# YAIconvalley/distributed-pipeline

Measured on AMD Instinct MI355X. Metric: train steps/sec (whole node), DiffuSeq-base seq128 DDP at 1/2/4/8 MI355X, higher is better.
Workload: dtype bf16

## Files before the change

distributed_pipeline_amd/csrc/bindings.cpp:

```cpp
#include <cstdlib>
#include <cstring>
#include <torch/extension.h>
#include <ATen/hip/impl/HIPStreamMasqueradingAsCUDA.h>
#include <c10/core/DeviceGuard.h>

#include <vector>

#include "launchers.h"

namespace dpa {
void register_comm(pybind11::module& m);
void register_runtime(pybind11::module& m);
}

#define CHECK_DEV(x) TORCH_CHECK((x).is_cuda(), #x " must be a HIP tensor")
#define CHECK_CONTIG(x) TORCH_CHECK((x).is_contiguous(), #x " must be contiguous")
#define CHECK_F32(x) TORCH_CHECK((x).scalar_type() == at::kFloat, #x " must be float32")
#define CHECK_BF16(x) TORCH_CHECK((x).scalar_type() == at::kBFloat16, #x " must be bfloat16")
#define CHECK_ALIGNED(x) \
  TORCH_CHECK(reinterpret_cast<uintptr_t>((x).data_ptr()) % 16 == 0, #x " must be 16-byte aligned")

static inline hipStream_t cur_stream() { return c10::hip::getCurrentHIPStreamMasqueradingAsCUDA().stream(); }

static void sqnorm(const at::Tensor& g, at::Tensor& partial, at::Tensor& out, double scale,
// ... 1207 lines not shown
        py::arg("part_buf") = py::none(), py::arg("part_acc") = false, py::arg("beta") = py::none(),
        py::arg("hcopy") = py::none(), py::arg("pair_hash") = false);
  m.def("colsum_acc", &colsum_acc, "dst += colsum(part) (fp32 partials [rows, cols])");
  m.def("ln_bwd_partials", &ln_bwd_partials, "floats of add_ln_bwd's deferred partial buffer (0: none)");
  m.def("ln_colreduce", &ln_colreduce, "dg/db(/dyb) += column sums of add_ln_bwd partials",
        py::arg("part"), py::arg("R"), py::arg("D"), py::arg("dg"), py::arg("db"), py::arg("dyb") = py::none());
  m.def("bias_act_fwd", &bias_act_fwd, "z += bias (in place); y = act(z) -> (z, y)");
  m.def("bias_act_bwd", &bias_act_bwd, "dz = dy*act'(zy); db = colsum(dz) -> (dz, db)");
  m.def("gemm_nt_into", &gemm_nt_into, "y = x W^T (+b) into a preallocated [T, N] tensor");
  m.def("gemm_nn_into", &gemm_nn_into, "dx = dy W into a preallocated [T, K] tensor");
  m.def("emb_grad", &emb_grad, "dW[ids] += dy (sorted segment sum, fp32)");
  m.def("id_sort", &id_sort, "counting sort of int64 ids into V + 1 buckets -> (sorted ids, permutation)");
  m.def("partition01", &partition01, "stable partition order of an int64 0/1 mask (nonzero first)");
  m.def("attn128_supports", &dpa::attn128_supports, "the persistent L = 128 attention covers (L, D, causal)");
  m.def("attn_fwd", &attn_fwd, "fused attention forward (head_dim 64/128) -> (out, lse)", py::arg("qkv"),
        py::arg("heads"), py::arg("p"), py::arg("causal"), py::arg("seed"), py::arg("offset"),
        py::arg("head_major") = false);
  m.def("attn_bwd", &attn_bwd, "fused attention backward -> (dqkv, colsum(dqkv) or None)",
        py::arg("dout"), py::arg("qkv"), py::arg("out"), py::arg("lse"), py::arg("heads"), py::arg("p"),
        py::arg("causal"), py::arg("seed"), py::arg("offset"), py::arg("want_db") = false,
        py::arg("head_major") = false, py::arg("db_acc") = py::none(), py::arg("part_out") = py::none());
  m.def("attn_colpart_rows", &dpa::attn_colpart_rows,
        "rows of attn_bwd's bias-gradient partials ([rows][3 D] fp32) for (B, L, H, D, causal)");
  m.def("attn_colpart_reduce", &attn_colpart_reduce,
        "db[3 H D] += column sums of R x H rows of attn_bwd partials (deferred bias gradient)");
  m.def("gemm_nt", &gemm_nt,
        "y = act(x W^T + b) (bf16 MFMA) -> (y, z, z_is_derivative): z is the pre-activation, or "
        "act'(pre-activation) when want_deriv and the persistent kernel ran (backward act code 4)",
        py::arg("x"), py::arg("W"), py::arg("b"), py::arg("act"), py::arg("want_deriv") = 0,
        py::arg("head_major_L") = 0);
  m.def("gemm_nt_res", &gemm_nt_res, "h = res + dropout_p(x W^T + b) in the GEMM epilogue (None: shape not tiled)",
        py::arg("x"), py::arg("W"), py::arg("b"), py::arg("res"), py::arg("p"), py::arg("seed"), py::arg("offset"));
  m.def("gemm_nn", &gemm_nn, "dx = dy W (bf16 MFMA; wt = W^T takes the row-form operand path)", py::arg("dy"),
        py::arg("W"), py::arg("wt") = py::none());
  m.def("gemm_nn_dact", &gemm_nn_dact,
        "dz = (dy W) * act'(aux) (bf16 MFMA, fused act backward) -> (dz, colsum(dz) fp32 or None)",
        py::arg("dy"), py::arg("W"), py::arg("aux"), py::arg("act"), py::arg("want_db") = false,
        py::arg("db_acc") = py::none(), py::arg("part_out") = py::none(), py::arg("wt") = py::none());
  m.def("gemm_nn_acc_", &gemm_nn_acc_, "dx += dy W in place (bf16 MFMA); False if the shape does not tile",
        py::arg("dy"), py::arg("W"), py::arg("dx"), py::arg("wt") = py::none());
  m.def("gemm_wgrad", &gemm_wgrad, "dW += dy^T x, db += colsum(dy) (fp32 atomics, split-K)");
  m.def("gemm_wgrad_multi", &gemm_wgrad_multi, "dW += sum_s dy_s^T x_s over equal token segments, one launch",
        py::arg("dys"), py::arg("xs"), py::arg("dW"), py::arg("db") = py::none());
  m.def("gemm_wgrad_grouped", &gemm_wgrad_grouped,
        "dW_i += sum_s dy_is^T x_is for several Linears in one launch (no token split); false if a site does not tile",
        py::arg("dys"), py::arg("xs"), py::arg("dWs"), py::arg("dbs"));
  m.def("gemm_supported", &gemm_supported, "shape check for the native GEMMs");
  m.def("set_gemm256", &dpa::set_gemm256, "enable/disable the 256x256 8-phase GEMM path");
  m.def("set_gemmp_grid_cap", &dpa::set_gemmp_grid_cap, "cap the persistent GEMM grid (0 = #CUs)");
  m.def("set_wgrad4w", &dpa::set_wgrad4w,
        "weight gradients without in-kernel bias sums on the one-wave-per-SIMD kernel (wgrad4w.hip; default on)");
  m.def("set_gemmp_half", &dpa::set_gemmp_half,
        "128-row tiles of the persistent GEMMs: 0 off, 1 auto (when they finish sooner), 2 always, -1 default");
  m.def("set_gemmp_dynamic", &dpa::set_gemmp_dynamic,
        "dynamic per-XCD tile queues for the persistent GEMMs (on for world > 1; env DPA_GEMMP_DYNAMIC wins)");
  m.def("linear_argmax", &linear_argmax,
        "row-wise arg-max of x W^T + c without the scores -> (idx int64, best fp32); ties: lowest index",
        py::arg("x"), py::arg("W"), py::arg("c") = py::none());
  m.def("row_half_sqnorm", &row_half_sqnorm, "c[v] = -1/2 ||W[v]||^2 in fp32 from a bf16 W");
  m.def("lxent_fwd", &lxent_fwd, "fused linear + cross-entropy forward -> (loss, lse)");
  m.def("lxent_fwd_dx", &lxent_fwd_dx,
        "fused linear-CE forward + unscaled input gradient -> (loss, lse, dxu fp32 [N, E])");
  m.def("lxent_bwd", &lxent_bwd, "fused linear + cross-entropy backward -> (dx, dW fp32, db fp32)",
        pybind11::arg("dloss"), pybind11::arg("x"), pybind11::arg("W"), pybind11::arg("b"), pybind11::arg("tgt"),
        pybind11::arg("lse"), pybind11::arg("need_dx"), pybind11::arg("need_dw"), pybind11::arg("need_db"),
        pybind11::arg("onehot_scatter") = false, pybind11::arg("dw_acc") = pybind11::none(),
        pybind11::arg("db_acc") = pybind11::none());
  m.def("seq_pos_sums", &seq_pos_sums, "(sum over b, sum over l) of a [B*L, H] bf16 gradient in one read",
        pybind11::arg("d"), pybind11::arg("L"), pybind11::arg("need_pos"), pybind11::arg("need_temb"));
  m.def("xent_rows_fwd", &xent_rows_fwd, "row softmax-CE over bf16 logits [R, ld] -> (loss, lse)",
        pybind11::arg("lg"), pybind11::arg("V"), pybind11::arg("tgt"), pybind11::arg("loss_out") = pybind11::none(),
        pybind11::arg("lse_out") = pybind11::none());
  m.def("xent_rows_bwd_", &xent_rows_bwd_, "in place: logits -> dloss * (softmax - onehot)");
  m.def("xent_rows_fwd_grad_", &xent_rows_fwd_grad_,
        "in place: logits -> softmax - onehot (unscaled), returns (loss, lse) or [] if the row is too long",
        pybind11::arg("lg"), pybind11::arg("V"), pybind11::arg("tgt"), pybind11::arg("loss_out") = pybind11::none(),
        pybind11::arg("lse_out") = pybind11::none());
  m.def("emb_qsample_fwd", &emb_qsample_fwd,
        "DiffuSeq embedding gather + x_start noise + masked q_sample -> (x_start, x_start bf16, x_t bf16)");
  m.def("reverse_step", &reverse_step,
        "DiffuSeq reverse update a x0 + a_prev x0_prev + b x + s z (in-kernel Philox noise; source rows kept) -> (out fp32, out bf16 | None)",
        py::arg("like"), py::arg("N"), py::arg("E"), py::arg("x") = py::none(), py::arg("pred") = py::none(),
        py::arg("idx") = py::none(), py::arg("W") = py::none(), py::arg("x_start") = py::none(),
        py::arg("mask") = py::none(), py::arg("scale") = 1.0, py::arg("a") = 0.0, py::arg("b") = 0.0,
        py::arg("s") = 0.0, py::arg("seed") = 0, py::arg("step") = 0, py::arg("row_base") = 0,
        py::arg("tau") = 0.0, py::arg("erf_tau") = 0.0, py::arg("want_bf16") = false,
        py::arg("pred_prev") = py::none(), py::arg("idx_prev") = py::none(), py::arg("a_prev") = 0.0);
  m.def("ngram_matches", &ngram_matches,
        "clipped 1..4-gram match counts of every sequence pair of a group -> int32 [G, K, K, 4] | None (shape not covered)",
        py::arg("tokens"), py::arg("lens"));
  m.def("lcs_lengths", &lcs_lengths,
        "longest-common-subsequence length of every sequence pair of a group -> int32 [G, K, K] | None (shape not covered)",
        py::arg("tokens"), py::arg("lens"));
  m.def("emb_qsample_bwd", &emb_qsample_bwd, "scatter-add of the q_sample gradients into dW (fp32)");
  m.def("diff_loss_fwd", &diff_loss_fwd, "DiffuSeq per-sample (mse, tT) losses");
  m.def("diff_loss_bwd", &diff_loss_bwd, "backward of diff_loss_fwd -> (d_out, d_x_start)", py::arg("xs"),
        py::arg("out"), py::arg("ids"), py::arg("t"), py::arg("W"), py::arg("dmse"), py::arg("dtT"),
        py::arg("sa_last"), py::arg("need_dout"), py::arg("need_dxs"), py::arg("dW"), py::arg("fold_t0") = false);
  m.def("rng_base_add", &rng_base_add, "advance the device-side Philox offset base (graph replays)");
  m.def("timestep_emb", &timestep_emb, "sinusoidal timestep embedding [cos | sin] -> bf16");
}
```

distributed_pipeline_amd/csrc/gemm256.hip:

```cpp
#include <cstdlib>

#include "act.h"
#include "common.h"
#include "launchers.h"
#include "mfma.h"

namespace dpa {
namespace g256 {

typedef __attribute__((address_space(3))) void lds_void;
typedef const __attribute__((address_space(1))) void glob_void;
typedef __attribute__((ext_vector_type(8))) __bf16 bf16x8_v;

constexpr int HALF = 16384;
constexpr int B_REGION = 65536;
__host__ __device__ constexpr int img_off(int buf, int h) { return buf * 2 * HALF + h * HALF; }

enum { EPI_BF16 = 0, EPI_BIAS_ACT = 1, EPI_ATOMIC_F32 = 2, EPI_DACT = 3, EPI_NONE = 4 };

__device__ __forceinline__ f32x4 mfma16(const bf16x8& a, const bf16x8& b, const f32x4& c) {
  return __builtin_amdgcn_mfma_f32_16x16x32_bf16(__builtin_bit_cast(bf16x8_v, a),
                                                 __builtin_bit_cast(bf16x8_v, b), c, 0, 0, 0);
}

__device__ __forceinline__ uint32_t lds_u32(const void* p) {
  return (uint32_t)reinterpret_cast<uintptr_t>((const __attribute__((address_space(3))) char*)p);
}

__device__ __forceinline__ int tr_x(int row) { return ((row & 3) << 1) | (((row >> 3) & 1) << 3); }

__device__ __forceinline__ float act_f(float z, int act) { return act_apply(z, act); }
__device__ __forceinline__ float dact_f(float a, int act) { return act_deriv(a, act); }

__device__ __forceinline__ void barrier() { asm volatile("s_barrier" ::: "memory"); }

template <bool TR>
struct Operand {
  const bf16_t* base;
  int64_t ld;
  uint32_t off[2];
  uint32_t rd[4];
  int wv;
  int hstep;

  __device__ __forceinline__ void init(const bf16_t* p, int64_t ld_, int row0, int w, int lane,
                                       int wsub, int wrows, uint32_t region, bool remap = false) {
    ld = ld_;
    wv = w;
    hstep = remap ? 32 : 128;
    base = TR ? p + row0 : p + (int64_t)row0 * ld_;
#pragma unroll
    for (int j = 0; j < 2; ++j) {
      const int piece = w * 2 + j;
// ... 528 lines not shown
  uint32_t o[4], g[4];
#pragma unroll
  for (int q = 0; q < 4; ++q) {
    f32x2 d;
    const f32x2 y = act_dact2<ACT>(f32x2{__uint_as_float(w[q] << 16), __uint_as_float(w[q] & 0xffff0000u)}, d);
    o[q] = pack_bf2(y.x, y.y);
    g[q] = pack_bf2(d.x, d.y);
  }
  dv = make_uint4(g[0], g[1], g[2], g[3]);
  return make_uint4(o[0], o[1], o[2], o[3]);
}

template <int ACT>
__device__ __forceinline__ uint4 act8(const uint4& u) {
  const uint32_t w[4] = {u.x, u.y, u.z, u.w};
  uint32_t o[4];
#pragma unroll
  for (int q = 0; q < 4; ++q) {
    const f32x2 y = act2<ACT>(f32x2{__uint_as_float(w[q] << 16), __uint_as_float(w[q] & 0xffff0000u)});
    o[q] = pack_bf2(y.x, y.y);
  }
  return make_uint4(o[0], o[1], o[2], o[3]);
}

constexpr float Q8_LO_STEP = 0.5f / 74.f;
#ifndef DPA_Q8_CVT
#define DPA_Q8_CVT 1
#endif
__device__ __forceinline__ f32x2 q8_codes2(f32x2 d) {
  const f32x2 l1 = d * 148.f + 19.f;
  const f32x2 l2 = d * 256.f - 35.f;
  f32x2 c = {fmaxf(l1.x, l2.x), fmaxf(l1.y, l2.y)};
  if constexpr (DPA_Q8_CVT == 0) c = f32x2{__builtin_rintf(c.x), __builtin_rintf(c.y)};
  return c;
}

template <int ACT>
__device__ __forceinline__ uint4 act_dact8q(const uint4& u, uint2& c) {
  const uint32_t w[4] = {u.x, u.y, u.z, u.w};
  uint32_t o[4], cw[2] = {0u, 0u};
#pragma unroll
  for (int q = 0; q < 4; ++q) {
    f32x2 d;
    const f32x2 y = act_dact2<ACT>(f32x2{__uint_as_float(w[q] << 16), __uint_as_float(w[q] & 0xffff0000u)}, d);
    o[q] = pack_bf2(y.x, y.y);
    const f32x2 cc = q8_codes2(d);
    cw[q >> 1] = __builtin_amdgcn_cvt_pk_u8_f32(cc.x, (q & 1) * 2, cw[q >> 1]);
    cw[q >> 1] = __builtin_amdgcn_cvt_pk_u8_f32(cc.y, (q & 1) * 2 + 1, cw[q >> 1]);
  }
  c = make_uint2(cw[0], cw[1]);
  return make_uint4(o[0], o[1], o[2], o[3]);
}

__device__ __forceinline__ f32x2 q8_pair(const uint4& a, int q) {
  const uint32_t c = (q >> 1) ? a.y : a.x;
  const int sh = (q & 1) * 16;
  const f32x2 cv = {(float)((c >> sh) & 0xffu), (float)((c >> (sh + 8)) & 0xffu)};
  const f32x2 lo = (cv - 19.f) * Q8_LO_STEP;
  const f32x2 hi = cv * (1.f / 256.f) + 35.f / 256.f;
  return f32x2{fminf(lo.x, hi.x), fminf(lo.y, hi.y)};
}

__device__ __forceinline__ void lds_write_b32(uint32_t addr, int v) {
  asm volatile("ds_write_b32 %0, %1\n\ts_waitcnt lgkmcnt(0)" ::"v"(addr), "v"(v) : "memory");
}
__device__ __forceinline__ int lds_read_b32_sync(uint32_t addr) {
  int v;
  asm volatile("ds_read_b32 %0, %1\n\ts_waitcnt lgkmcnt(0)" : "=v"(v) : "v"(addr) : "memory");
  return v;
}

__device__ __forceinline__ float bf_lo(uint32_t w) { return __uint_as_float(w << 16); }
__device__ __forceinline__ float bf_hi(uint32_t w) { return __uint_as_float(w & 0xffff0000u); }

#ifndef DPA_GEMM_EARLY_AUX
#define DPA_GEMM_EARLY_AUX 1
#endif
constexpr int PEARLY_AUX = DPA_GEMM_EARLY_AUX;

template <int POL>
__device__ __forceinline__ void st_out(bf16_t* p, const uint4& v) {
  if constexpr (POL & 4) {
    const u32x4_v x = {v.x, v.y, v.z, v.w};
    asm volatile("global_store_dwordx4 %0, %1, off sc1\n\ts_nop 1" ::"v"(p), "v"(x) : "memory");
  } else if constexpr (POL & 1) {
    const u32x4_v x = {v.x, v.y, v.z, v.w};
    __builtin_nontemporal_store(x, reinterpret_cast<u32x4_v*>(p));
  } else {
    *reinterpret_cast<uint4*>(p) = v;
  }
}
template <int POL>
__device__ __forceinline__ uint4 ld_aux(const bf16_t* p) {
  if constexpr (POL & 2) {
    const u32x4_v x = __builtin_nontemporal_load(reinterpret_cast<const u32x4_v*>(p));
    return make_uint4(x[0], x[1], x[2], x[3]);
  } else {
    return *reinterpret_cast<const uint4*>(p);
  }
}
typedef __attribute__((ext_vector_type(2))) unsigned u32x2_v;
template <int POL>
__device__ __forceinline__ void st_out8(uint8_t* p, const uint2& v) {
  if constexpr (POL & 1) {
    __builtin_nontemporal_store(u32x2_v{v.x, v.y}, reinterpret_cast<u32x2_v*>(p));
  } else {
    *reinterpret_cast<uint2*>(p) = v;
  }
}
template <int POL>
__device__ __forceinline__ uint2 ld_aux8(const uint8_t* p) {
  if constexpr (POL & 2) {
    const u32x2_v x = __builtin_nontemporal_load(reinterpret_cast<const u32x2_v*>(p));
    return make_uint2(x[0], x[1]);
  } else {
    return *reinterpret_cast<const uint2*>(p);
  }
}

struct EpiArgs {
  uint32_t seed = 0, offset = 0, thr16 = 0;
  float scale = 1.f;
};

template <int GM>
__device__ __forceinline__ void tile_mn(int t, int NT, int& mt, int& nt) {
  if constexpr (GM <= 1) {
    mt = t / NT;
    nt = t - mt * NT;
  } else {
    const int gs = GM * NT, g = t / gs, r = t - g * gs;
    mt = g * GM + r % GM;
    nt = r / GM;
  }
}

template <bool B_TR, int EPI, int ACT, int POL = 0, int GM = 1, int STG = 0, int DU = 0, bool HMT = false>
__global__ void __launch_bounds__(512) gemmp_kernel(const bf16_t* __restrict__ A, int64_t lda,
                                                    const bf16_t* __restrict__ B, int64_t ldb, int M, int N,
                                                    int nk, bf16_t* __restrict__ C, int64_t ldc,
                                                    const bf16_t* __restrict__ bias,
                                                    bf16_t* __restrict__ Zout, float* __restrict__ colpart,
                                                    int* __restrict__ tile_ctr, int hm, EpiArgs ea) {
  __shared__ __attribute__((aligned(1024))) char smem[P_LDS];
  static_assert(!(HMT && EPI == 4), "column-sum partials are laid out per 256-row tile");
  constexpr int TM = HMT ? 128 : 256, NRO = HMT ? 4 : 8;
  constexpr int XS = HMT ? PEpi<EPI>::XS_H : PEpi<EPI>::XS;
  constexpr bool DACT = EPI == 3 || EPI == 4 || EPI == 5;
  constexpr bool AUXR = DACT || EPI == 7;
  constexpr bool Q8 = DACT && ACT == 5;
  static_assert(!(EPI == 8 && ACT == 0), "EPI 8 stores an activation derivative");
  const int w = __builtin_amdgcn_readfirstlane(threadIdx.x >> 6);
  const int wm = (w >> 2) & 1, wn = w & 3;
  const int grp = w >> 2;
  const int NT = N / 256, ntiles = (M / TM) * NT;
  const int G = gridDim.x;
  const uint32_t sbase = lds_u32(smem);
  char* const smB = smem + B_REGION;
  const int niter = nk >> 1;
  const bool has_bias = bias != nullptr;

  Operand<false> opA;
  Operand<B_TR> opB;
  f32x4 acc[2][2][4][2];
  bf16x8 fa[4][2], fb0[2][2], fb1[2][2];
  float cs = 0.f;
  const uint32_t csa[2] = {0u, 0u};

  auto prologue = [&](int t, int slot) {
    int mt, nt;
    tile_mn<GM>(t, NT, mt, nt);
    const int lane = lane_id();
    opA.init(A, lda, mt * TM, w, lane, wm, 64, sbase);
    if constexpr (HMT) opA.hstep = 0;
    opB.init(B, ldb, nt * 256, w, lane, wn, 32, sbase + B_REGION, true);
    const int bh = (w & 1) * 256;
    const char* bsrc = (has_bias ? reinterpret_cast<const char*>(bias + nt * 256)
                                 : reinterpret_cast<const char*>(A)) + bh + lane * 4;
    __builtin_amdgcn_global_load_lds((glob_void*)bsrc, (lds_void*)(smem + P_BIAS_OFF + slot * 512 + bh),
                                     4, 0, 0);
    opA.stage(smem + img_off(0, 0), 0, 0);
    opB.stage(smB + img_off(0, 0), 0, 0);
    opB.stage(smB + img_off(0, 1), 1, 0);
    opA.stage(smem + img_off(0, 1), 1, 0);
    opA.stage(smem + img_off(1, 0), 0, 1);
    opB.stage(smB + img_off(1, 0), 0, 1);
  };

  auto row_off = [&](int t, int ro, int k, int ln) -> int64_t {
    int mt, nt;
    tile_mn<GM>(t, NT, mt, nt);
    const int qa = ro >> 2, i = ro & 3;
    const int lrow = qa * 128 + wm * 64 + i * 16 + k * 8 + (ln >> 3);
    const int col = nt * 256 + wn * 64 + (ln & 7) * 8;
    if (EPI == 0 && hm) {
      const int64_t row = (int64_t)mt * TM + lrow;
      const int64_t b = row >> hm, l = row & ((1 << hm) - 1);
// ... 68 lines not shown
      }
      if constexpr (AUXR) {
        if (ro == 0) {
          if (has_next) wait_vm<15>(); else wait_vm<2>();
        } else if (ro == 1) {
          if (has_next) wait_vm<17>(); else wait_vm<4>();
        } else if (ro < NRO - 1) {
          wait_vm<6>();
        } else {
          wait_vm<4>();
        }
        uint32_t rA = 0, cB = 0;
        if constexpr (EPI == 7) {
          int mt, nt;
          tile_mn<GM>(t, NT, mt, nt);
          rA = (uint32_t)(mt * TM + qa * 128 + wm * 64 + i * 16 + (ln >> 3)) * 0x9E3779B1u;
          cB = (uint32_t)((nt * 256 + wn * 64 + (ln & 7) * 8) >> 1) * 0x85EBCA77u;
        }
#pragma unroll
        for (int k = 0; k < 2; ++k) {
          const uint4 a = aux[ro & 1][k];
          const uint32_t aw[4] = {a.x, a.y, a.z, a.w};
          const uint32_t vw[4] = {val[k].x, val[k].y, val[k].z, val[k].w};
          uint32_t o[4];
#pragma unroll
          for (int q = 0; q < 4; ++q) {
            const f32x2 x = f32x2{bf_lo(vw[q]), bf_hi(vw[q])};
            f32x2 d;
            if constexpr (Q8) {
              d = x * q8_pair(a, q);
            } else if constexpr (EPI == 7) {
              const f32x2 r = f32x2{bf_lo(aw[q]), bf_hi(aw[q])};
              const uint32_t hsh = mix32(dsm ^ (rA + (uint32_t)k * (8u * 0x9E3779B1u)) ^
                                         (cB + (uint32_t)q * 0x85EBCA77u));
              const f32x2 m = {(hsh & 0xffffu) >= ea.thr16 ? ea.scale : 0.f, (hsh >> 16) >= ea.thr16 ? ea.scale : 0.f};
              d = x * m + r;
            } else {
              const f32x2 av = f32x2{bf_lo(aw[q]), bf_hi(aw[q])};
              d = EPI == 5 ? x + av : x * dact2<ACT>(av);
            }
            o[q] = pack_bf2(d.x, d.y);
            if constexpr (EPI == 4) {
              csum[2 * q] += bf_lo(o[q]);
              csum[2 * q + 1] += bf_hi(o[q]);
            }
          }
          val[k] = make_uint4(o[0], o[1], o[2], o[3]);
        }
        if (ro + 2 < NRO) {
#pragma unroll
          for (int k = 0; k < 2; ++k) aux[ro & 1][k] = load_aux(t, ro + 2, k, ln);
        }
      }
#pragma unroll
      for (int k = 0; k < 2; ++k) {
        const int64_t o = row_off(t, ro, k, ln);
        if constexpr (EPI == 2) st_out<POL>(Zout + o, val[k]);
        if constexpr (EPI == 1 || EPI == 2) val[k] = act8<ACT>(val[k]);
        if constexpr (EPI == 6) {
          uint4 dv;
          val[k] = act_dact8<ACT>(val[k], dv);
          st_out<POL>(Zout + o, dv);
        }
        if constexpr (EPI == 8) {
          uint2 code;
          val[k] = act_dact8q<ACT>(val[k], code);
          st_out8<POL>(reinterpret_cast<uint8_t*>(Zout) + q8_off(t, ro, k, ln), code);
        }
        st_out<POL>(C + o, val[k]);
      }
    }
    if constexpr (EPI == 4) {
#pragma unroll
      for (int e = 0; e < 8; ++e) {
        float x = csum[e];
        x += __int_as_float(__builtin_amdgcn_update_dpp(0, __float_as_int(x), 0x128, 0xF, 0xF, true));
        x += __shfl_xor(x, 16, 64);
        x += __shfl_xor(x, 32, 64);
        csum[e] = x;
      }
      int mt, nt;
    tile_mn<GM>(t, NT, mt, nt);
      float* dst = colpart + ((int64_t)mt * 2 + wm) * (int64_t)(NT * 256) + nt * 256 + wn * 64 + ch * 8;
      if (ln < 8) {
        *reinterpret_cast<float4*>(dst) = make_float4(csum[0], csum[1], csum[2], csum[3]);
        *reinterpret_cast<float4*>(dst + 4) = make_float4(csum[4], csum[5], csum[6], csum[7]);
      }
    }
  };

  int tile = xcd_remap(blockIdx.x, G);
  if (tile >= ntiles) return;
  const bool dyn = tile_ctr != nullptr && G >= 8;
  int qbase = 0, qsize = 1;
  int* qctr = nullptr;
  if (dyn) {
    const int qg = G >> 3, rg = G & 7, x = blockIdx.x & 7;
    qbase = x < rg ? x * (qg + 1) : rg * (qg + 1) + (x - rg) * qg;
    qsize = x < rg ? qg + 1 : qg;
    qctr = tile_ctr + x * 16;
  }
  int slot = 0;
  bool extra = false;
  if constexpr (STG > 1) {
    const int ph = (blockIdx.x >> 3) % STG;
    for (int i = 0; i < ph * DU; ++i) __builtin_amdgcn_s_sleep(32);
  }
  prologue(tile, slot);
  wait_vm<8>();
  barrier();
  if (grp == 1) barrier();

  while (true) {
    int claimed = 0;
    if (dyn && w == 0 && lane_id() == 0) claimed = atomicAdd(qctr, 1);
    {
      const bool more = 1 < niter;
      phase<0, false, B_TR, false, true, XS, 0, HMT, true>(acc, fa, fb0, fb1, cs, opA, opB, smem, csa, 0, more, false, grp, extra);
      phase<1, false, B_TR, false, true, XS, 0, HMT, true>(acc, fa, fb0, fb1, cs, opA, opB, smem, csa, 0, more, false, grp, extra);
      phase<2, false, B_TR, false, true, XS, 0, HMT, true>(acc, fa, fb0, fb1, cs, opA, opB, smem, csa, 0, more, false, grp, extra);
      phase<3, false, B_TR, false, true, XS, 0, HMT, true>(acc, fa, fb0, fb1, cs, opA, opB, smem, csa, 0, more, false, grp, extra);
      phase<4, false, B_TR, false, true, 0, 0, HMT>(acc, fa, fb0, fb1, cs, opA, opB, smem, csa, 0, more, false, grp);
      phase<5, false, B_TR, false, true, 0, 0, HMT>(acc, fa, fb0, fb1, cs, opA, opB, smem, csa, 0, more, false, grp);
      phase<6, false, B_TR, false, true, 0, 0, HMT>(acc, fa, fb0, fb1, cs, opA, opB, smem, csa, 0, more, false, grp);
      phase<7, false, B_TR, false, true, 0, 0, HMT>(acc, fa, fb0, fb1, cs, opA, opB, smem, csa, 0, more, false, grp);
    }
    uint4 aux[2][2];
    constexpr bool EARLY_AUX = AUXR && (PEARLY_AUX != 0);
    for (int it = 1; it < niter - (EARLY_AUX ? 1 : 0); ++it) {
      const int te = 2 * it;
      const bool more = it + 1 < niter;
      phase<0, false, B_TR, false, true, 0, 0, HMT>(acc, fa, fb0, fb1, cs, opA, opB, smem, csa, te, more, false, grp);
      phase<1, false, B_TR, false, true, 0, 0, HMT>(acc, fa, fb0, fb1, cs, opA, opB, smem, csa, te, more, false, grp);
      phase<2, false, B_TR, false, true, 0, 0, HMT>(acc, fa, fb0, fb1, cs, opA, opB, smem, csa, te, more, false, grp);
      phase<3, false, B_TR, false, true, 0, 0, HMT>(acc, fa, fb0, fb1, cs, opA, opB, smem, csa, te, more, false, grp);
      phase<4, false, B_TR, false, true, 0, 0, HMT>(acc, fa, fb0, fb1, cs, opA, opB, smem, csa, te, more, false, grp);
      phase<5, false, B_TR, false, true, 0, 0, HMT>(acc, fa, fb0, fb1, cs, opA, opB, smem, csa, te, more, false, grp);
      phase<6, false, B_TR, false, true, 0, 0, HMT>(acc, fa, fb0, fb1, cs, opA, opB, smem, csa, te, more, false, grp);
      phase<7, false, B_TR, false, true, 0, 0, HMT>(acc, fa, fb0, fb1, cs, opA, opB, smem, csa, te, more, false, grp);
    }
    bool aux_issued = false;
    if constexpr (EARLY_AUX) {
      if (niter > 1) {
        const int te = 2 * (niter - 1);
        phase<0, false, B_TR, false, true, 0, 0, HMT>(acc, fa, fb0, fb1, cs, opA, opB, smem, csa, te, false, false, grp);
        phase<1, false, B_TR, false, true, 0, 0, HMT>(acc, fa, fb0, fb1, cs, opA, opB, smem, csa, te, false, false, grp);
        {
          const int ln = opaque(lane_id());
#pragma unroll
          for (int ro = 0; ro < 2; ++ro)
#pragma unroll
            for (int k = 0; k < 2; ++k) aux[ro][k] = load_aux(tile, ro, k, ln);
        }
        aux_issued = true;
        phase<2, false, B_TR, false, true, 0, 4, HMT>(acc, fa, fb0, fb1, cs, opA, opB, smem, csa, te, false, false, grp);
        phase<3, false, B_TR, false, true, 0, 4, HMT>(acc, fa, fb0, fb1, cs, opA, opB, smem, csa, te, false, false, grp);
        phase<4, false, B_TR, false, true, 0, 4, HMT>(acc, fa, fb0, fb1, cs, opA, opB, smem, csa, te, false, false, grp);
        phase<5, false, B_TR, false, true, 0, 4, HMT>(acc, fa, fb0, fb1, cs, opA, opB, smem, csa, te, false, false, grp);
        phase<6, false, B_TR, false, true, 0, 4, HMT>(acc, fa, fb0, fb1, cs, opA, opB, smem, csa, te, false, false, grp);
        phase<7, false, B_TR, false, true, 0, 4, HMT>(acc, fa, fb0, fb1, cs, opA, opB, smem, csa, te, false, false, grp);
      }
// ... 110 lines not shown
  int* slot = q->buf + (size_t)q->cursor * SLOT_INTS;
  q->cursor = (q->cursor + 1) % NSLOT;
  return slot;
}

template <bool B_TR, int EPI, int ACT, int POL = 0, int GM = 1, bool HMT = false>
static void gemmp_launch(const uint16_t* a, int64_t lda, const uint16_t* b, int64_t ldb, int M, int N, int K,
                         uint16_t* c, const uint16_t* bias, uint16_t* z, int ncu, hipStream_t s,
                         float* colpart, int hm, const g256::EpiArgs& ea) {
  const int tiles = (M / (HMT ? 128 : 256)) * (N / 256);
  const int grid = persistent_grid(tiles, ncu);
  int* q = (tiles > grid && grid >= 8) ? gemmp_queue(s) : nullptr;
  hipLaunchKernelGGL((g256::gemmp_kernel<B_TR, EPI, ACT, POL, GM, 0, 0, HMT>), dim3(grid), dim3(512), 0, s,
                     (const bf16_t*)a, lda, (const bf16_t*)b, ldb, M, N, K / 64, (bf16_t*)c, (int64_t)N,
                     (const bf16_t*)bias, (bf16_t*)z, colpart, q, hm, ea);
}

static int g_gemmp_half = -1;
void set_gemmp_half(int mode) { g_gemmp_half = mode < 0 ? -1 : mode; }
static bool use_half_tiles(int M, int N, int ncu) {
  if (g_gemmp_half < 0) {
    const char* e = std::getenv("DPA_GEMMP_HALF");
    g_gemmp_half = e ? std::atoi(e) : 1;
  }
  const int mode = g_gemmp_half;
  constexpr double HALF_COST = 0.66;
  if (mode == 0 || M % 256) return false;
  if (mode >= 2) return true;
  const int g = persistent_grid(1 << 30, ncu);
  const int t = (M / 256) * (N / 256);
  const int rf = (t + g - 1) / g, rh = (2 * t + g - 1) / g;
  return rh * HALF_COST < rf * 0.97;
}

template <bool B_TR, int EPI, int ACT>
static void gemmp_go(const uint16_t* a, int64_t lda, const uint16_t* b, int64_t ldb, int M, int N, int K,
                     uint16_t* c, const uint16_t* bias, uint16_t* z, int ncu, hipStream_t s,
                     float* colpart = nullptr, int hm = 0, const g256::EpiArgs& ea = g256::EpiArgs{}) {
  if constexpr (EPI != 4) {
    if (use_half_tiles(M, N, ncu)) {
      gemmp_launch<B_TR, EPI, ACT, 0, 1, true>(a, lda, b, ldb, M, N, K, c, bias, z, ncu, s, colpart, hm, ea);
      return;
    }
  }
  if constexpr (EPI == 4 || EPI == 6 || EPI == 8) {
    if ((M / 256) % 8 == 0 && N / 256 >= 8) {
      gemmp_launch<B_TR, EPI, ACT, 1, 8>(a, lda, b, ldb, M, N, K, c, bias, z, ncu, s, colpart, hm, ea);
      return;
    }
  }
  gemmp_launch<B_TR, EPI, ACT>(a, lda, b, ldb, M, N, K, c, bias, z, ncu, s, colpart, hm, ea);
}

bool launch_gemmp_nt(const uint16_t* x, const uint16_t* W, const uint16_t* bias, uint16_t* y,
                     uint16_t* z, int T, int N, int K, int act, int ncu, hipStream_t s, bool zderiv, int hm,
                     bool z8) {
  if (!g256_enabled() || T % 256 || N % 256 || K % 128 || K < 128 || act < 0 || act > 3 || N >= (1 << 24))
    return false;
  if (hm && (act != 0 || hm < 7 || hm > 30 || (T & ((1 << hm) - 1)) || N % 64)) return false;
  if (z8 && (act == 0 || z == nullptr || !zderiv)) return false;
  if (act == 0) gemmp_go<false, 0, 0>(x, K, W, K, T, N, K, y, bias, nullptr, ncu, s, nullptr, hm);
  else if (z8) {
    if (act == 1) gemmp_go<false, 8, 1>(x, K, W, K, T, N, K, y, bias, z, ncu, s);
    else if (act == 2) gemmp_go<false, 8, 2>(x, K, W, K, T, N, K, y, bias, z, ncu, s);
    else gemmp_go<false, 8, 3>(x, K, W, K, T, N, K, y, bias, z, ncu, s);
  } else if (z != nullptr && zderiv) {
    if (act == 1) gemmp_go<false, 6, 1>(x, K, W, K, T, N, K, y, bias, z, ncu, s);
    else if (act == 2) gemmp_go<false, 6, 2>(x, K, W, K, T, N, K, y, bias, z, ncu, s);
    else gemmp_go<false, 6, 3>(x, K, W, K, T, N, K, y, bias, z, ncu, s);
  } else if (z == nullptr) {
    if (act == 1) gemmp_go<false, 1, 1>(x, K, W, K, T, N, K, y, bias, nullptr, ncu, s);
    else if (act == 2) gemmp_go<false, 1, 2>(x, K, W, K, T, N, K, y, bias, nullptr, ncu, s);
    else gemmp_go<false, 1, 3>(x, K, W, K, T, N, K, y, bias, nullptr, ncu, s);
  } else {
    if (act == 1) gemmp_go<false, 2, 1>(x, K, W, K, T, N, K, y, bias, z, ncu, s);
    else if (act == 2) gemmp_go<false, 2, 2>(x, K, W, K, T, N, K, y, bias, z, ncu, s);
    else gemmp_go<false, 2, 3>(x, K, W, K, T, N, K, y, bias, z, ncu, s);
  }
  return true;
}

bool launch_gemmp_nt_res(const uint16_t* x, const uint16_t* W, const uint16_t* bias, const uint16_t* res,
                         uint16_t* h, int T, int N, int K, int ncu, hipStream_t s, float p, uint32_t seed,
                         uint32_t offset) {
  if (!g256_enabled() || T % 256 || N % 256 || K % 128 || K < 128 || !(p >= 0.f && p < 1.f) || N >= (1 << 24))
    return false;
  g256::EpiArgs ea;
  ea.seed = seed;
  ea.offset = offset;
  ea.thr16 = pair_thr16(p);
  ea.scale = 1.f / (1.f - p);
  gemmp_go<false, 7, 0>(x, K, W, K, T, N, K, h, bias, const_cast<uint16_t*>(res), ncu, s, nullptr, 0, ea);
  return true;
}

template <int EPI, int ACT>
static void gemmp_dgrad(const uint16_t* dy, const uint16_t* W, const uint16_t* WT, int T, int N, int K,
                        uint16_t* dx, uint16_t* z, int ncu, hipStream_t s, float* colpart = nullptr) {
  if (WT != nullptr)
    gemmp_go<false, EPI, ACT>(dy, N, WT, N, T, K, N, dx, nullptr, z, ncu, s, colpart);
  else
    gemmp_go<true, EPI, ACT>(dy, N, W, K, T, K, N, dx, nullptr, z, ncu, s, colpart);
}

bool launch_gemmp_nn_acc(const uint16_t* dy, const uint16_t* W, uint16_t* dx, int T, int N, int K, int ncu,
                         hipStream_t s, const uint16_t* WT) {
  if (!g256_enabled() || T % 256 || K % 256 || N % 128 || N < 128 || K >= (1 << 24)) return false;
  gemmp_dgrad<5, 0>(dy, W, WT, T, N, K, dx, dx, ncu, s);
  return true;
}

bool launch_gemmp_nn(const uint16_t* dy, const uint16_t* W, uint16_t* dx, const uint16_t* aux, int act,
                     int T, int N, int K, int ncu, hipStream_t s, float* colpart, const uint16_t* WT) {
  if (!g256_enabled() || T % 256 || K % 256 || N % 128 || N < 128 || act < 0 || act > 5 || K >= (1 << 24))
    return false;
  uint16_t* ax = const_cast<uint16_t*>(aux);
  if (act == 0 || aux == nullptr) {
    if (colpart) return false;
// ... 172 lines not shown
```

distributed_pipeline_amd/csrc/launchers.h:

```cpp
#pragma once
#include <hip/hip_runtime.h>
#include <stdint.h>

namespace dpa {

constexpr int IPC_MAXW = 8;
struct IpcPeers {
  float* stage[IPC_MAXW];
  uint32_t* flags[IPC_MAXW];
};
struct IpcData {
  float* p[IPC_MAXW];
};
constexpr int64_t IPC_FLAG_WORDS = 4 * 1024;
int ipc_allreduce_blocks(int64_t n, int W, bool two_shot);
bool launch_ipc_allreduce(const IpcPeers& peers, const IpcData& data, int W, int rank, int sim_ranks,
                          int64_t n, int64_t cap, uint32_t epoch, bool two_shot, int* err, hipStream_t s);

void launch_comm_sim(void* buf, int64_t bytes, int64_t touch_bytes, uint64_t ticks, int cus,
                     unsigned long long* tl, hipStream_t s);
void launch_time_marker(unsigned long long* slot, hipStream_t s);
void launch_comm_sim_stats(const unsigned long long* tl, int nb, const unsigned long long* bwd_end,
                           unsigned long long* acc, hipStream_t s);

// ... 107 lines not shown
                            uint16_t* x_start16, uint16_t* x_t, hipStream_t s);
int64_t emb_grad_part_floats(int64_t NT, int E, bool qsample);
bool launch_emb_grad(const int64_t* sorted_ids, const int64_t* perm, const float* dy32, const uint16_t* dy16,
                     int64_t NT, int E, int V, float* dW, float* part, hipStream_t s);
bool launch_emb_qsample_bwd(const int64_t* ids, const int64_t* mask, const int64_t* t, const float* sa,
                            const float* d_xs, const uint16_t* d_xs16, const uint16_t* d_xt16,
                            const float* d_xt32, int64_t NT, int L, int E, int V, float* dW,
                            hipStream_t s, const int64_t* sorted_ids = nullptr,
                            const int64_t* perm = nullptr, float* part = nullptr);
bool launch_diff_loss_fwd(const float* x_start, const void* out, bool out_bf16, const int64_t* ids,
                          const int64_t* t, const float* W, int B, int L, int E, int V, float sa_last,
                          float* mse, float* tT, hipStream_t s);
bool launch_diff_loss_bwd(const float* x_start, const void* out, bool out_bf16, const int64_t* ids,
                          const int64_t* t, const float* W, const float* dmse, const float* dtT, int B,
                          int L, int E, int V, float sa_last, void* d_out, float* d_xs, float* dW,
                          hipStream_t s, bool fold_t0 = false);
void launch_timestep_emb(const float* ts, int B, int dim, float max_period, uint16_t* out,
                         hipStream_t s);

bool launch_reverse_step(const float* x, const uint16_t* pred, const int64_t* idx, const float* W,
                         const float* x_start, const int64_t* mask, int64_t N, int E, int V, float scale,
                         float a, float b, float s, uint64_t seed, uint32_t step, uint64_t row_base,
                         float tau, float erf_tau, float* out, uint16_t* out16, hipStream_t st,
                         const uint16_t* pred_prev = nullptr, const int64_t* idx_prev = nullptr,
                         float a_prev = 0.f);

bool launch_ngram_match(const void* tokens, bool tok64, const int* lens, int64_t G, int K, int L, int* m,
                        hipStream_t st);

bool launch_lcs_lengths(const void* tokens, bool tok64, const int* lens, int64_t G, int K, int L, int* out,
                        hipStream_t st);

int64_t id_sort_workspace_ints(int64_t n, int V);
bool launch_id_bucket_sort(const int64_t* ids, int64_t n, int V, int* ws, int64_t* sorted, int64_t* perm,
                           hipStream_t s);
int64_t partition01_workspace_ints(int64_t n);
bool launch_partition01(const int64_t* mask, int64_t n, int* blk_ws, int64_t* order, hipStream_t s);

bool launch_gemm_nt(const uint16_t* x, const uint16_t* W, const uint16_t* bias, uint16_t* y,
                    uint16_t* z, int T, int N, int K, int act, hipStream_t s,
                    bool* zderiv = nullptr, int hm = 0);
bool launch_gemm_nn(const uint16_t* dy, const uint16_t* W, uint16_t* dx, int T, int N, int K,
                    hipStream_t s, const uint16_t* WT = nullptr);
bool launch_gemm_wgrad(const uint16_t* dy, const uint16_t* x, float* dW, float* db, int T, int N,
                       int K, hipStream_t s, float* ws = nullptr);
bool launch_gemm256_nt(const uint16_t* x, const uint16_t* W, const uint16_t* bias, uint16_t* y,
                       uint16_t* z, int T, int N, int K, int act, hipStream_t s);
bool launch_gemm256_nn(const uint16_t* dy, const uint16_t* W, uint16_t* dx, int T, int N, int K,
                       hipStream_t s);
void set_gemm256(bool on);
void set_gemmp_dynamic(bool on);
void set_gemmp_grid_cap(int cap);
void set_gemmp_half(int mode);
bool launch_gemm256_nn_dact(const uint16_t* dy, const uint16_t* W, const uint16_t* aux,
                            uint16_t* dz, int T, int N, int K, int act, hipStream_t s);
bool launch_gemm256_wgrad(const uint16_t* dy, const uint16_t* x, float* dW, float* db, int T,
                          int N, int K, hipStream_t s, float* ws = nullptr);
int64_t gemm256_wgrad_workspace_floats(int T, int N, int K, int nseg = 1);
bool launch_gemm256_wgrad_multi(const uint16_t* const* dys, const uint16_t* const* xs, int nseg, float* dW,
                                float* db, int T, int N, int K, hipStream_t s, float* ws);
struct WgGroupSite {
  const uint16_t* a[8];
  const uint16_t* b[8];
  float* dW;
  float* colsum;
  int nseg, M, N, ktiles, tile0, pad[3];
};
int wgrad_group_prepare(WgGroupSite* sites, int nsites);
bool launch_wgrad_group(const WgGroupSite* d_sites, int nsites, int ntiles, hipStream_t s);
bool launch_gemmp_nt(const uint16_t* x, const uint16_t* W, const uint16_t* bias, uint16_t* y,
                     uint16_t* z, int T, int N, int K, int act, int ncu, hipStream_t s,
                     bool zderiv = false, int hm = 0, bool z8 = false);
bool launch_gemmp_nt_res(const uint16_t* x, const uint16_t* W, const uint16_t* bias, const uint16_t* res,
                         uint16_t* h, int T, int N, int K, int ncu, hipStream_t s, float p, uint32_t seed,
                         uint32_t offset);
bool launch_gemmp_nn(const uint16_t* dy, const uint16_t* W, uint16_t* dx, const uint16_t* aux, int act,
                     int T, int N, int K, int ncu, hipStream_t s, float* colpart, const uint16_t* WT = nullptr);
bool launch_gemmp_nn_acc(const uint16_t* dy, const uint16_t* W, uint16_t* dx, int T, int N, int K, int ncu,
                         hipStream_t s, const uint16_t* WT = nullptr);
int device_cu_count();
void rng_base_add_attention(uint32_t d, hipStream_t s);
void rng_base_add_attention128(uint32_t d, hipStream_t s);
void rng_base_add_diffusion(uint32_t d, hipStream_t s);
void rng_base_add_norm(uint32_t d, hipStream_t s);
void rng_base_add_gemm256(uint32_t d, hipStream_t s);

}
```

Measured before the change: 6.178.

## Compute forward GEMM activation and u8 derivative codes via LDS lookup table

Adds a precomputed per-device table mapping bf16 pre-activations in a bounded exponent range to the activation output and its 8-bit derivative code. The EPI 8 persistent GEMM epilogue copies the table into extra LDS and replaces the per-element transcendental activation math with gathered ds_read lookups. Small-magnitude values are patched with a linear shortcut, and waves holding out-of-range values fall back to the exact path. The cost is more LDS per block, which may lower occupancy, plus a table load in each block prologue and a one-time table build that synchronizes the stream.

```diff
diff --git a/distributed_pipeline_amd/csrc/bindings.cpp b/distributed_pipeline_amd/csrc/bindings.cpp
--- a/distributed_pipeline_amd/csrc/bindings.cpp
+++ b/distributed_pipeline_amd/csrc/bindings.cpp
@@ -1283,6 +1283,11 @@
         "weight gradients without in-kernel bias sums on the one-wave-per-SIMD kernel (wgrad4w.hip; default on)");
   m.def("set_gemmp_half", &dpa::set_gemmp_half,
         "128-row tiles of the persistent GEMMs: 0 off, 1 auto (when they finish sooner), 2 always, -1 default");
+  m.def("get_gemmp_act_table", &dpa::get_gemmp_act_table, "whether the EPI 8 activation table is on");
+  m.def("gemmp_act_table_built", &dpa::gemmp_act_table_built,
+        "whether the current device holds the EPI 8 activation table of this activation code", py::arg("act"));
+  m.def("set_gemmp_act_table", &dpa::set_gemmp_act_table,
+        "u8-act' forward GEMM epilogue (gemm_nt want_deriv=2): activation by LDS table lookup (env DPA_GEMM_ACT_TABLE)");
   m.def("set_gemmp_dynamic", &dpa::set_gemmp_dynamic,
         "dynamic per-XCD tile queues for the persistent GEMMs (on for world > 1; env DPA_GEMMP_DYNAMIC wins)");
   m.def("linear_argmax", &linear_argmax,
diff --git a/distributed_pipeline_amd/csrc/gemm256.hip b/distributed_pipeline_amd/csrc/gemm256.hip
--- a/distributed_pipeline_amd/csrc/gemm256.hip
+++ b/distributed_pipeline_amd/csrc/gemm256.hip
@@ -1,4 +1,5 @@
 #include <cstdlib>
+#include <mutex>
 
 #include "act.h"
 #include "common.h"
@@ -633,6 +634,65 @@
   return make_uint4(o[0], o[1], o[2], o[3]);
 }
 
+constexpr int ACT_TAB_ENTRIES = 2 * 14 * 128;
+constexpr int ACT_TAB_BYTES = ACT_TAB_ENTRIES * 4;
+constexpr uint32_t ACT_TAB_SMALL = 0x3980u, ACT_TAB_END = 0x4080u;
+constexpr int p_lds_bytes(int epi) { return P_LDS + (epi == 8 ? ACT_TAB_BYTES : 0); }
+static_assert(p_lds_bytes(8) <= 160 * 1024 && P_LDS >= 8 * (int)ACT_TAB_SMALL, "activation table placement");
+
+template <int ACT>
+__global__ void __launch_bounds__(64) act_table_kernel(uint32_t* __restrict__ tab) {
+  const int i = blockIdx.x * 64 + threadIdx.x;
+  if (i >= ACT_TAB_ENTRIES / 8) return;
+  uint32_t zw[4];
+#pragma unroll
+  for (int q = 0; q < 4; ++q) {
+    const uint32_t a = 0x3A80u + (uint32_t)(4 * i + q);
+    zw[q] = a | ((a | 0x8000u) << 16);
+  }
+  uint2 c;
+  const uint4 y = act_dact8q<ACT>(make_uint4(zw[0], zw[1], zw[2], zw[3]), c);
+  const uint32_t yw[4] = {y.x, y.y, y.z, y.w}, cw[2] = {c.x, c.y};
+#pragma unroll
+  for (int e = 0; e < 8; ++e)
+    tab[8 * i + e] = ((yw[e >> 1] >> (16 * (e & 1))) & 0xffffu) | (((cw[e >> 2] >> (8 * (e & 3))) & 0xffu) << 16);
+}
+
+typedef __attribute__((ext_vector_type(2))) unsigned short u16x2_v;
+typedef __attribute__((ext_vector_type(2))) short i16x2_v;
+__device__ __forceinline__ uint32_t pk_sub_u16(uint32_t a, uint32_t b) {
+  return __builtin_bit_cast(uint32_t, __builtin_bit_cast(u16x2_v, a) - __builtin_bit_cast(u16x2_v, b));
+}
+__device__ __forceinline__ uint32_t pk_max_u16(uint32_t a, uint32_t b) {
+  return __builtin_bit_cast(uint32_t, __builtin_elementwise_max(__builtin_bit_cast(u16x2_v, a), __builtin_bit_cast(u16x2_v, b)));
+}
+__device__ __forceinline__ uint32_t pk_min_u16(uint32_t a, uint32_t b) {
+  return __builtin_bit_cast(uint32_t, __builtin_elementwise_min(__builtin_bit_cast(u16x2_v, a), __builtin_bit_cast(u16x2_v, b)));
+}
+__device__ __forceinline__ uint32_t pk_sign_i16(uint32_t a) {
+  return __builtin_bit_cast(uint32_t, __builtin_bit_cast(i16x2_v, a) >> (short)15);
+}
+
+template <int OFF>
+__device__ __forceinline__ void act_tab_gather8(uint32_t (&t)[8], const uint32_t (&a)[8]) {
+  static_assert(OFF >= 0 && OFF < 65536, "ds_read offset field");
+  asm volatile(
+      "ds_read_b32 %0, %8 offset:%16\n\tds_read_b32 %1, %9 offset:%16\n\t"
+      "ds_read_b32 %2, %10 offset:%16\n\tds_read_b32 %3, %11 offset:%16\n\t"
+      "ds_read_b32 %4, %12 offset:%16\n\tds_read_b32 %5, %13 offset:%16\n\t"
+      "ds_read_b32 %6, %14 offset:%16\n\tds_read_b32 %7, %15 offset:%16"
+      : "=&v"(t[0]), "=&v"(t[1]), "=&v"(t[2]), "=&v"(t[3]), "=&v"(t[4]), "=&v"(t[5]), "=&v"(t[6]), "=&v"(t[7])
+      : "v"(a[0]), "v"(a[1]), "v"(a[2]), "v"(a[3]), "v"(a[4]), "v"(a[5]), "v"(a[6]), "v"(a[7]), "i"(OFF)
+      : "memory");
+}
+__device__ __forceinline__ void act_tab_wait(uint32_t (&t)[16]) {
+  asm volatile("s_waitcnt lgkmcnt(0)"
+               : "+v"(t[0]), "+v"(t[1]), "+v"(t[2]), "+v"(t[3]), "+v"(t[4]), "+v"(t[5]), "+v"(t[6]), "+v"(t[7]),
+                 "+v"(t[8]), "+v"(t[9]), "+v"(t[10]), "+v"(t[11]), "+v"(t[12]), "+v"(t[13]), "+v"(t[14]), "+v"(t[15])
+               :
+               : "memory");
+}
+
 __device__ __forceinline__ f32x2 q8_pair(const uint4& a, int q) {
   const uint32_t c = (q >> 1) ? a.y : a.x;
   const int sh = (q & 1) * 16;
@@ -702,6 +762,7 @@
 struct EpiArgs {
   uint32_t seed = 0, offset = 0, thr16 = 0;
   float scale = 1.f;
+  const uint32_t* act_tab = nullptr;
 };
 
 template <int GM>
@@ -723,7 +784,7 @@
                                                     const bf16_t* __restrict__ bias,
                                                     bf16_t* __restrict__ Zout, float* __restrict__ colpart,
                                                     int* __restrict__ tile_ctr, int hm, EpiArgs ea) {
-  __shared__ __attribute__((aligned(1024))) char smem[P_LDS];
+  __shared__ __attribute__((aligned(1024))) char smem[p_lds_bytes(EPI)];
   static_assert(!(HMT && EPI == 4), "column-sum partials are laid out per 256-row tile");
   constexpr int TM = HMT ? 128 : 256, NRO = HMT ? 4 : 8;
   constexpr int XS = HMT ? PEpi<EPI>::XS_H : PEpi<EPI>::XS;
@@ -898,6 +959,63 @@
           for (int k = 0; k < 2; ++k) aux[ro & 1][k] = load_aux(t, ro + 2, k, ln);
         }
       }
+      [[maybe_unused]] uint2 code8[2];
+      if constexpr (EPI == 8) {
+        bool looked_up = false;
+        if (ea.act_tab != nullptr) {
+          const uint32_t vw[8] = {val[0].x, val[0].y, val[0].z, val[0].w, val[1].x, val[1].y, val[1].z, val[1].w};
+          uint32_t e[8], emax = 0u, emin = 0xffffffffu;
+#pragma unroll
+          for (int p = 0; p < 8; ++p) {
+            e[p] = pk_sub_u16(vw[p] & 0x7fff7fffu, 0x01000100u);
+            emax = pk_max_u16(emax, e[p]);
+            emin = pk_min_u16(emin, e[p]);
+          }
+          const bool out = max(emax & 0xffffu, emax >> 16) >= ACT_TAB_END;
+          if (__builtin_amdgcn_ballot_w64(out) == 0) {
+            constexpr int TAB0 = P_LDS - 8 * (int)ACT_TAB_SMALL;
+            uint32_t ad[16], tv[16];
+#pragma unroll
+            for (int p = 0; p < 8; ++p) {
+              ad[2 * p] = sbase + ((e[p] & 0xffffu) << 3) + ((vw[p] >> 13) & 4u);
+              ad[2 * p + 1] = sbase + ((e[p] >> 16) << 3) + ((vw[p] >> 29) & 4u);
+            }
+            act_tab_gather8<TAB0>(reinterpret_cast<uint32_t(&)[8]>(tv[0]), reinterpret_cast<const uint32_t(&)[8]>(ad[0]));
+            act_tab_gather8<TAB0>(reinterpret_cast<uint32_t(&)[8]>(tv[8]), reinterpret_cast<const uint32_t(&)[8]>(ad[8]));
+            act_tab_wait(tv);
+            uint32_t yw[8], cw[4];
+#pragma unroll
+            for (int p = 0; p < 8; ++p) yw[p] = __builtin_amdgcn_perm(tv[2 * p + 1], tv[2 * p], 0x05040100u);
+#pragma unroll
+            for (int h = 0; h < 4; ++h)
+              cw[h] = __builtin_amdgcn_perm(tv[4 * h + 1], tv[4 * h], 0x0c0c0602u) |
+                      __builtin_amdgcn_perm(tv[4 * h + 3], tv[4 * h + 2], 0x06020c0cu);
+            const bool small = min(emin & 0xffffu, emin >> 16) < ACT_TAB_SMALL;
+            if (__builtin_amdgcn_ballot_w64(small) != 0) {
+              uint32_t sm[8];
+#pragma unroll
+              for (int p = 0; p < 8; ++p) {
+                sm[p] = pk_sign_i16(pk_sub_u16(e[p], ACT_TAB_SMALL * 0x10001u));
+                yw[p] = (yw[p] & ~sm[p]) | (pk_sub_u16(vw[p], 0x00800080u) & sm[p]);
+              }
+#pragma unroll
+              for (int h = 0; h < 4; ++h) {
+                const uint32_t bm = __builtin_amdgcn_perm(sm[2 * h + 1], sm[2 * h], 0x06040200u);
+                cw[h] = (cw[h] & ~bm) | (0x5d5d5d5du & bm);
+              }
+            }
+            val[0] = make_uint4(yw[0], yw[1], yw[2], yw[3]);
+            val[1] = make_uint4(yw[4], yw[5], yw[6], yw[7]);
+            code8[0] = make_uint2(cw[0], cw[1]);
+            code8[1] = make_uint2(cw[2], cw[3]);
+            looked_up = true;
+          }
+        }
+        if (!looked_up) {
+#pragma unroll
+          for (int k = 0; k < 2; ++k) val[k] = act_dact8q<ACT>(val[k], code8[k]);
+        }
+      }
 #pragma unroll
       for (int k = 0; k < 2; ++k) {
         const int64_t o = row_off(t, ro, k, ln);
@@ -909,9 +1027,7 @@
           st_out<POL>(Zout + o, dv);
         }
         if constexpr (EPI == 8) {
-          uint2 code;
-          val[k] = act_dact8q<ACT>(val[k], code);
-          st_out8<POL>(reinterpret_cast<uint8_t*>(Zout) + q8_off(t, ro, k, ln), code);
+          st_out8<POL>(reinterpret_cast<uint8_t*>(Zout) + q8_off(t, ro, k, ln), code8[k]);
         }
         st_out<POL>(C + o, val[k]);
       }
@@ -953,6 +1069,17 @@
     for (int i = 0; i < ph * DU; ++i) __builtin_amdgcn_s_sleep(32);
   }
   prologue(tile, slot);
+  if constexpr (EPI == 8) {
+    if (ea.act_tab != nullptr) {
+      uint32_t tv[ACT_TAB_ENTRIES / 512];
+#pragma unroll
+      for (int i = 0; i < ACT_TAB_ENTRIES / 512; ++i) tv[i] = ea.act_tab[i * 512 + (int)threadIdx.x];
+#pragma unroll
+      for (int i = 0; i < ACT_TAB_ENTRIES / 512; ++i)
+        lds_write_b32(sbase + P_LDS + (uint32_t)(i * 512 + (int)threadIdx.x) * 4, (int)tv[i]);
+      wait_vm<0>();
+    }
+  }
   wait_vm<8>();
   barrier();
   if (grp == 1) barrier();
@@ -1169,6 +1296,53 @@
   gemmp_launch<B_TR, EPI, ACT>(a, lda, b, ldb, M, N, K, c, bias, z, ncu, s, colpart, hm, ea);
 }
 
+#ifndef DPA_GEMM_ACT_TABLE_DEFAULT
+#define DPA_GEMM_ACT_TABLE_DEFAULT 1
+#endif
+static int g_gemmp_act_table = -1;
+void set_gemmp_act_table(bool on) { g_gemmp_act_table = on ? 1 : 0; }
+bool get_gemmp_act_table() {
+  if (g_gemmp_act_table < 0) {
+    const char* e = std::getenv("DPA_GEMM_ACT_TABLE");
+    g_gemmp_act_table = e ? (e[0] == '0' ? 0 : 1) : DPA_GEMM_ACT_TABLE_DEFAULT;
+  }
+  return g_gemmp_act_table != 0;
+}
+constexpr int ACT_TAB_MAXDEV = 64;
+static uint32_t* g_act_tabs[ACT_TAB_MAXDEV][2];
+static std::mutex g_act_tabs_mu;
+bool gemmp_act_table_built(int act) {
+  int dev = 0;
+  if ((act != 1 && act != 3) || hipGetDevice(&dev) != hipSuccess || dev < 0 || dev >= ACT_TAB_MAXDEV) return false;
+  std::lock_guard<std::mutex> lock(g_act_tabs_mu);
+  return g_act_tabs[dev][act == 3] != nullptr;
+}
+static const uint32_t* gemmp_act_table(int act, hipStream_t s) {
+  if (!get_gemmp_act_table() || (act != 1 && act != 3)) return nullptr;
+  int dev = 0;
+  if (hipGetDevice(&dev) != hipSuccess || dev < 0 || dev >= ACT_TAB_MAXDEV) return nullptr;
+  std::lock_guard<std::mutex> lock(g_act_tabs_mu);
+  uint32_t*& tab = g_act_tabs[dev][act == 3];
+  if (tab != nullptr) return tab;
+  hipStreamCaptureStatus cs = hipStreamCaptureStatusNone;
+  if (hipStreamIsCapturing(s, &cs) != hipSuccess || cs != hipStreamCaptureStatusNone) return nullptr;
+  uint32_t* buf = nullptr;
+  if (hipMalloc(&buf, g256::ACT_TAB_BYTES) != hipSuccess) {
+    (void)hipGetLastError();
+    return nullptr;
+  }
+  constexpr int blocks = (g256::ACT_TAB_ENTRIES / 8 + 63) / 64;
+  if (act == 1) hipLaunchKernelGGL(g256::act_table_kernel<1>, dim3(blocks), dim3(64), 0, s, buf);
+  else hipLaunchKernelGGL(g256::act_table_kernel<3>, dim3(blocks), dim3(64), 0, s, buf);
+  if (hipGetLastError() != hipSuccess || hipStreamSynchronize(s) != hipSuccess) {
+    (void)hipGetLastError();
+    (void)hipFree(buf);
+    return nullptr;
+  }
+  tab = buf;
+  return tab;
+}
+
 bool launch_gemmp_nt(const uint16_t* x, const uint16_t* W, const uint16_t* bias, uint16_t* y,
                      uint16_t* z, int T, int N, int K, int act, int ncu, hipStream_t s, bool zderiv, int hm,
                      bool z8) {
@@ -1178,9 +1352,11 @@
   if (z8 && (act == 0 || z == nullptr || !zderiv)) return false;
   if (act == 0) gemmp_go<false, 0, 0>(x, K, W, K, T, N, K, y, bias, nullptr, ncu, s, nullptr, hm);
   else if (z8) {
-    if (act == 1) gemmp_go<false, 8, 1>(x, K, W, K, T, N, K, y, bias, z, ncu, s);
-    else if (act == 2) gemmp_go<false, 8, 2>(x, K, W, K, T, N, K, y, bias, z, ncu, s);
-    else gemmp_go<false, 8, 3>(x, K, W, K, T, N, K, y, bias, z, ncu, s);
+    g256::EpiArgs ea;
+    ea.act_tab = gemmp_act_table(act, s);
+    if (act == 1) gemmp_go<false, 8, 1>(x, K, W, K, T, N, K, y, bias, z, ncu, s, nullptr, 0, ea);
+    else if (act == 2) gemmp_go<false, 8, 2>(x, K, W, K, T, N, K, y, bias, z, ncu, s, nullptr, 0, ea);
+    else gemmp_go<false, 8, 3>(x, K, W, K, T, N, K, y, bias, z, ncu, s, nullptr, 0, ea);
   } else if (z != nullptr && zderiv) {
     if (act == 1) gemmp_go<false, 6, 1>(x, K, W, K, T, N, K, y, bias, z, ncu, s);
     else if (act == 2) gemmp_go<false, 6, 2>(x, K, W, K, T, N, K, y, bias, z, ncu, s);
diff --git a/distributed_pipeline_amd/csrc/launchers.h b/distributed_pipeline_amd/csrc/launchers.h
--- a/distributed_pipeline_amd/csrc/launchers.h
+++ b/distributed_pipeline_amd/csrc/launchers.h
@@ -183,6 +183,9 @@
 void set_gemmp_dynamic(bool on);
 void set_gemmp_grid_cap(int cap);
 void set_gemmp_half(int mode);
+bool get_gemmp_act_table();
+bool gemmp_act_table_built(int act);
+void set_gemmp_act_table(bool on);
 bool launch_gemm256_nn_dact(const uint16_t* dy, const uint16_t* W, const uint16_t* aux,
                             uint16_t* dz, int T, int N, int K, int act, hipStream_t s);
 bool launch_gemm256_wgrad(const uint16_t* dy, const uint16_t* x, float* dW, float* db, int T,
```

New measurement: 6.235 (median of 6 runs). No clear change (+0.9%).
